# FedeMont/collision_handling_in_instantNGP

Hardware: AMD Instinct MI355X
Metric: Mpixels/sec fwd+bwd at L=16,F=2,T=2^19 (higher is better)
Workload: dtype f32

## Files before the change

collision_handling_in_instantngp_amd/csrc/decoder.hip:

```cpp
#include "gngf_common.h"
#include <type_traits>
#include <utility>

namespace gngf {

using f32x16 = __attribute__((ext_vector_type(16))) float;

constexpr int kH = 64;
constexpr int kDecThreads = 256;

__device__ __forceinline__ int crow(int r, int h) { return (r & 3) + 8 * (r >> 2) + 4 * h; }
__device__ __forceinline__ int kmapC(int s2, int h) { return 32 * (s2 >> 4) + crow(s2 & 15, h); }

__device__ __forceinline__ float vmax0(float z) { float r; asm("v_max_f32 %0, 0, %1" : "=v"(r) : "v"(z)); return r; }
template <bool LEAKY> __device__ __forceinline__ float hidden_act(float z) {
  if (LEAKY) { float r; const float t = 0.01f * z; asm("v_max_f32 %0, %1, %2" : "=v"(r) : "v"(z), "v"(t)); return r; }
  return vmax0(z);
}
template <bool LEAKY> __device__ __forceinline__ float hidden_dsel(float y, float d) { return y > 0.f ? d : (LEAKY ? 0.01f * d : 0.f); }

using f32x2 = __attribute__((ext_vector_type(2))) float;
__device__ __forceinline__ unsigned lds_addr(const float* p) {
  return (unsigned)(size_t)(__attribute__((address_space(3))) const float*)p;
}
// ... 405 lines not shown
  const int64_t ntiles = (P + 127) / 128;
  int64_t zlo = 0, zhi = 0;
  int zper = 0;
  constexpr bool kClears = TRAIN || (KIN == 64 && EXACT && !HYB);
  if constexpr (kClears) {
    if (zero_fill && zero_vecs > 0) {
      const int64_t per = (zero_vecs + gridDim.x - 1) / gridDim.x;
      zlo = (int64_t)blockIdx.x * per + threadIdx.x;
      zhi = (int64_t)(blockIdx.x + 1) * per < zero_vecs ? (int64_t)(blockIdx.x + 1) * per : zero_vecs;
      const int64_t my_tiles = (ntiles - blockIdx.x + gridDim.x - 1) / gridDim.x;
      zper = (int)((per + (int64_t)kDecThreads * my_tiles - 1) / ((int64_t)kDecThreads * my_tiles));
    }
  }
  const unsigned xoff = (unsigned)(((wave * 32 + i) * in_dim + (EXACT ? h * S0 : 0)) * 4);
  const unsigned yoff = (unsigned)(((wave * 32 + i) * out_dim) * 4);
  float xr[S0], yn[4], dyn[4], dz3[4];
  const bool fused_loss = target != nullptr;
  const float* dsrc = fused_loss ? target : dY;
  const float kloss = fused_loss ? gloss[0] * (2.0f / (float)(P * out_dim)) : 0.f;
  auto tile_window = [&](int64_t t, int64_t& tt, int& rows) {
    tt = t < ntiles ? bwd_tile(t, ntiles) : ntiles;
    int64_t rem = P - tt * 128;
    rows = (int)(rem < 0 ? 0 : (rem > 128 ? 128 : rem));
  };
  auto fetch_x = [&](int64_t t) {
    int64_t tt; int rows;
    tile_window(t, tt, rows);
    const __amdgpu_buffer_rsrc_t rx = __builtin_amdgcn_make_buffer_rsrc(const_cast<float*>(X) + tt * 128 * in_dim, 0, rows * in_dim * 4, 0x00020000);
    if (EXACT) {
#pragma unroll
      for (int k = 0; k < S0 / 4; ++k) {
        const u32x4 v = __builtin_amdgcn_raw_buffer_load_b128(rx, xoff + 16 * k, 0, GNGF_BWD_X_AUX);
        xr[4 * k] = __uint_as_float(v.x); xr[4 * k + 1] = __uint_as_float(v.y);
        xr[4 * k + 2] = __uint_as_float(v.z); xr[4 * k + 3] = __uint_as_float(v.w);
      }
    } else {
#pragma unroll
      for (int sx = 0; sx < S0; ++sx) {
        const int k = h * S0 + sx;
        xr[sx] = __uint_as_float(__builtin_amdgcn_raw_buffer_load_b32(rx, k < in_dim ? xoff + 4 * k : 0x40000000u, 0, 0));
      }
    }
  };
  auto fetch_y = [&](int64_t t) {
    int64_t tt; int rows;
    tile_window(t, tt, rows);
    const __amdgpu_buffer_rsrc_t ry = __builtin_amdgcn_make_buffer_rsrc(const_cast<float*>(Yout) + tt * 128 * out_dim, 0, rows * out_dim * 4, 0x00020000);
    const __amdgpu_buffer_rsrc_t rd = __builtin_amdgcn_make_buffer_rsrc(const_cast<float*>(dsrc) + tt * 128 * out_dim, 0, rows * out_dim * 4, 0x00020000);
#pragma unroll
    for (int c = 0; c < 4; ++c) {
      const unsigned off = c < out_dim ? yoff + 4u * c : 0x40000000u;
      if constexpr (!TRAIN) yn[c] = __uint_as_float(__builtin_amdgcn_raw_buffer_load_b32(ry, off, 0, 0));
      dyn[c] = __uint_as_float(__builtin_amdgcn_raw_buffer_load_b32(rd, off, 0, 0));
    }
  };
  auto make_dz3 = [&]() {
#pragma unroll
    for (int c = 0; c < 4; ++c) {
      const float dy = fused_loss ? kloss * (yn[c] - dyn[c]) : dyn[c];
      dz3[c] = dy * (yn[c] * (1.f - yn[c]));
      asm volatile("" : "+v"(dz3[c]));
      db2acc[c] += dz3[c];
    }
  };
  fetch_x(blockIdx.x);
  fetch_y(blockIdx.x);
  if constexpr (!TRAIN) make_dz3();
  float b2v[4] = {0.f, 0.f, 0.f, 0.f};
  if constexpr (TRAIN) {
#pragma unroll
    for (int c = 0; c < 4; ++c) b2v[c] = raw[ro.b2 + c];
  }
  f32x16 b0v[2], b1v[2];
  if (RECOMPUTE) {
#pragma unroll
    for (int t = 0; t < 2; ++t) {
#pragma unroll
      for (int r = 0; r < 16; ++r) { b0v[t][r] = bs[32 * t + crow(r, h)]; b1v[t][r] = bs[kH + 32 * t + crow(r, h)]; }
      asm volatile("" : "+a"(b0v[t]), "+a"(b1v[t]));
    }
  }
  unsigned dxmax = 0u;
#if defined(GNGF_STAMPS)
  unsigned long long ph[10] = {0, 0, 0, 0, 0, 0, 0, 0, 0, 0}, tlast;
  asm volatile("s_memtime %0\n\ts_waitcnt lgkmcnt(0)" : "=s"(tlast) :: "memory");
#endif
  constexpr bool kCarryF0 = KIN <= 32;
  float f0[2][S0];
  f32x16 acc1[2], acc2[2];
  float ft[2][32];
  const unsigned hoff = (unsigned)(wave * 8192 + lane * 16);
  if (!RECOMPUTE && !TRAIN) {
    hidden_load(hidden, blockIdx.x, ntiles, 0, hoff, acc1);
    hidden_load(hidden, blockIdx.x, ntiles, 1, hoff, acc2);
    if constexpr (!HYB) {
#pragma unroll
      for (int s2 = 0; s2 < 32; ++s2) { ft[0][s2] = A1T[(0 * 32 + s2) * 64 + lane]; ft[1][s2] = A1T[(1 * 32 + s2) * 64 + lane]; }
    }
  }
  auto store_hidden_images = [&](auto E) {
    constexpr int e0 = 2 * E.value;
    static_for<2>([&](auto J) {
      constexpr int e = e0 + J.value, t = e >> 4, r = e & 15;
      lds_store<(32 * t + (r & 3) + 8 * (r >> 2)) * kImgStride * 4>(wTile, acc2[t][r]);
      lds_store<kImgB + (32 * t + (r & 3) + 8 * (r >> 2)) * kImgStride * 4>(wTile, acc1[t][r]);
    });
  };
  if constexpr (HYB && !TRAIN) static_for<16>([&](auto E) { store_hidden_images(E); });
  const u32x4* w1t = reinterpret_cast<const u32x4*>(A1T) + lane;
  const u32x4* w0t = reinterpret_cast<const u32x4*>(A0T) + lane;
  Planes w1p[HYB ? 8 : 1], w0p[HYB ? 4 : 1];
  if constexpr (HYB) {
#pragma unroll
    for (int f = 0; f < 8; ++f) {
      w1p[f] = load_planes(w1t + f * 3 * 64);
      asm volatile("" : "+a"(w1p[f].hi), "+a"(w1p[f].mid), "+a"(w1p[f].lo));
    }
  }
  u32x4* w1f = reinterpret_cast<u32x4*>(A1T);
  if constexpr (TRAIN) {
    asm volatile("s_waitcnt lgkmcnt(0)" ::: "memory");
    __syncthreads();
    for (int f = threadIdx.x >> 6; f < 8; f += 4) {
      const int cc = f >> 1, t = f & 1;
      const float* r1 = raw + ro.w1 + (32 * t + i) * 65;
      store_planes(w1f + f * 3 * 64 + lane, split8(r1[kmapS(cc, h, 0)], r1[kmapS(cc, h, 1)], r1[kmapS(cc, h, 2)], r1[kmapS(cc, h, 3)],
                                                  r1[kmapS(cc, h, 4)], r1[kmapS(cc, h, 5)], r1[kmapS(cc, h, 6)], r1[kmapS(cc, h, 7)]));
    }
    __syncthreads();
  }
  if (RECOMPUTE && kCarryF0) {
#pragma unroll
    for (int sx = 0; sx < S0; ++sx) { f0[0][sx] = A0[(0 * S0 + sx) * 64 + lane]; f0[1][sx] = A0[(1 * S0 + sx) * 64 + lane]; }
  }
#define STEP_END() __builtin_amdgcn_sched_barrier(0)
  for (int64_t tile = blockIdx.x; tile < ntiles; tile += gridDim.x) {
    pin_acc();
    STAMP(0);
    float f1[2][32];
    if constexpr (TRAIN) {
      Planes pa0 = load_planes(w0f + lane), pa1 = load_planes(w0f + 3 * 64 + lane);
#pragma unroll
      for (int t = 0; t < 2; ++t)
#pragma unroll
        for (int g = 0; g < 4; ++g) {
          const f32x4 q0 = *reinterpret_cast<const f32x4*>(bs + 32 * t + 8 * g + 4 * h);
          const f32x4 q1 = *reinterpret_cast<const f32x4*>(bs + kH + 32 * t + 8 * g + 4 * h);
#pragma unroll
          for (int e = 0; e < 4; ++e) { acc1[t][4 * g + e] = q0[e]; acc2[t][4 * g + e] = q1[e]; }
        }
      Planes zc = split8(xr[0], xr[1], xr[2], xr[3], xr[4], xr[5], xr[6], xr[7]);
      unsigned nh[4], nm[4], nl[4];
      auto quarter = [&](int q, float a, float b) {
        nh[q] = pack_hi16(b, a);
        const float ra = trunc_residual(a), rb = trunc_residual(b);
        nm[q] = pack_hi16(rb, ra);
        nl[q] = pack_hi16(trunc_residual(rb), trunc_residual(ra));
      };
      auto take_next = [&]() {
        zc.hi = u32x4{nh[0], nh[1], nh[2], nh[3]}; zc.mid = u32x4{nm[0], nm[1], nm[2], nm[3]}; zc.lo = u32x4{nl[0], nl[1], nl[2], nl[3]};
      };
      {
        const Planes na0 = load_planes(w0f + 2 * 3 * 64 + lane), na1 = load_planes(w0f + 3 * 3 * 64 + lane);
        acc1[0] = mfma_b(pa0.hi, zc.lo, acc1[0]);  acc1[1] = mfma_b(pa1.hi, zc.lo, acc1[1]);  quarter(0, xr[8], xr[9]);   STEP_END();
        acc1[0] = mfma_b(pa0.lo, zc.hi, acc1[0]);  acc1[1] = mfma_b(pa1.lo, zc.hi, acc1[1]);  quarter(1, xr[10], xr[11]); STEP_END();
        acc1[0] = mfma_b(pa0.mid, zc.mid, acc1[0]); acc1[1] = mfma_b(pa1.mid, zc.mid, acc1[1]); quarter(2, xr[12], xr[13]); STEP_END();
        acc1[0] = mfma_b(pa0.hi, zc.mid, acc1[0]); acc1[1] = mfma_b(pa1.hi, zc.mid, acc1[1]); quarter(3, xr[14], xr[15]); STEP_END();
        acc1[0] = mfma_b(pa0.mid, zc.hi, acc1[0]); acc1[1] = mfma_b(pa1.mid, zc.hi, acc1[1]);
        acc1[0] = mfma_b(pa0.hi, zc.hi, acc1[0]);  acc1[1] = mfma_b(pa1.hi, zc.hi, acc1[1]);  STEP_END();
        take_next(); pa0 = na0; pa1 = na1;
      }
      {
        const Planes na0 = load_planes(w1f + lane), na1 = load_planes(w1f + 3 * 64 + lane);
        mfma_split2(pa0, pa1, zc, acc1[0], acc1[1]);
        STEP_END();
        pa0 = na0; pa1 = na1;
      }
#pragma unroll
      for (int t = 0; t < 2; ++t)
#pragma unroll
        for (int r = 0; r < 16; ++r) acc1[t][r] = hidden_act<LEAKY>(acc1[t][r]);
      zc = split8(acc1[0][0], acc1[0][1], acc1[0][2], acc1[0][3], acc1[0][4], acc1[0][5], acc1[0][6], acc1[0][7]);
      STEP_END();
      static_for<4>([&](auto CC) {
        constexpr int cc = CC.value, nc = cc + 1;
        Planes na0, na1;
        if constexpr (nc < 4) { na0 = load_planes(w1f + (2 * nc) * 3 * 64 + lane); na1 = load_planes(w1f + (2 * nc + 1) * 3 * 64 + lane); }
        auto step = [&](auto PP, u32x4 a0, u32x4 a1, u32x4 b) {
          constexpr int pp = PP.value;
          acc2[0] = mfma_b(a0, b, acc2[0]);
          acc2[1] = mfma_b(a1, b, acc2[1]);
          if constexpr (nc < 4 && pp < 4) {
            constexpr int t = nc >> 1, r0 = 8 * (nc & 1) + 2 * pp;
            quarter(pp, acc1[t][r0], acc1[t][r0 + 1]);
          }
          if constexpr (pp < 4) {
            static_for<2>([&](auto E) {
              constexpr int e = 8 * cc + 2 * pp + E.value, tt = e >> 4, r = e & 15;
              lds_store<kImgB + (32 * tt + (r & 3) + 8 * (r >> 2)) * kImgStride * 4>(wTile, acc1[tt][r]);
            });
          }
          STEP_END();
        };
        step(std::integral_constant<int, 0>{}, pa0.hi, pa1.hi, zc.lo);
        step(std::integral_constant<int, 1>{}, pa0.lo, pa1.lo, zc.hi);
        step(std::integral_constant<int, 2>{}, pa0.mid, pa1.mid, zc.mid);
        step(std::integral_constant<int, 3>{}, pa0.hi, pa1.hi, zc.mid);
        step(std::integral_constant<int, 4>{}, pa0.mid, pa1.mid, zc.hi);
        step(std::integral_constant<int, 5>{}, pa0.hi, pa1.hi, zc.hi);
        if constexpr (nc < 4) { take_next(); pa0 = na0; pa1 = na1; }
      });
      f32x4 w2v[8];
#pragma unroll
      for (int g = 0; g < 8; ++g) w2v[g] = *reinterpret_cast<const f32x4*>(w2L + (g * 64 + lane) * 4);
#pragma unroll
      for (int t = 0; t < 2; ++t)
#pragma unroll
        for (int r = 0; r < 16; ++r) acc2[t][r] = hidden_act<LEAKY>(acc2[t][r]);
      STEP_END();
      {
        f32x4 o0 = {0.f, 0.f, 0.f, 0.f}, o1 = {0.f, 0.f, 0.f, 0.f};
#pragma unroll
        for (int g = 0; g < 8; ++g) {
          const f32x4 w = w2v[g];
          o0 = __builtin_amdgcn_mfma_f32_4x4x1f32(w.x, acc2[(4 * g) >> 4][(4 * g) & 15], o0, 0, 0, 0);
          o1 = __builtin_amdgcn_mfma_f32_4x4x1f32(w.y, acc2[(4 * g + 1) >> 4][(4 * g + 1) & 15], o1, 0, 0, 0);
          o0 = __builtin_amdgcn_mfma_f32_4x4x1f32(w.z, acc2[(4 * g + 2) >> 4][(4 * g + 2) & 15], o0, 0, 0, 0);
          o1 = __builtin_amdgcn_mfma_f32_4x4x1f32(w.w, acc2[(4 * g + 3) >> 4][(4 * g + 3) & 15], o1, 0, 0, 0);
        }
        int64_t rem = (P - tile * 128) * out_dim * 4;
        rem = rem > 128 * out_dim * 4 ? 128 * out_dim * 4 : rem;
        const __amdgpu_buffer_rsrc_t rs = __builtin_amdgcn_make_buffer_rsrc(const_cast<float*>(Yout) + tile * 128 * out_dim, 0, (int)rem, 0x00020000);
#pragma unroll
        for (int c = 0; c < 4; ++c) {
          const float dc = o0[c] + o1[c];
          const float z = dc + __shfl_xor(dc, 32, 64) + b2v[c];
          const float y = __builtin_amdgcn_rcpf(1.0f + __builtin_amdgcn_exp2f(z * -1.4426950408889634f));
          const unsigned off = (h == 0 && c < out_dim) ? yoff + 4u * c : 0x40000000u;
          __builtin_amdgcn_raw_buffer_store_b32(__float_as_uint(y), rs, off, 0, 0);
          yn[c] = (c < out_dim && tile * 128 + wave * 32 + i < P) ? y : 0.f;
        }
      }
      make_dz3();
      STEP_END();
    }
    if constexpr (RECOMPUTE) {
    if (!kCarryF0) {
#pragma unroll
      for (int sx = 0; sx < S0; ++sx) { f0[0][sx] = A0[(0 * S0 + sx) * 64 + lane]; f0[1][sx] = A0[(1 * S0 + sx) * 64 + lane]; }
      STEP_END();
    }
    static_for<S0>([&](auto SX) {
      constexpr int sx = SX.value;
      if constexpr (sx == 0) { acc1[0] = MFMA(f0[0][0], xr[0], b0v[0]); acc1[1] = MFMA(f0[1][0], xr[0], b0v[1]); }
      else { acc1[0] = MFMA(f0[0][sx], xr[sx], acc1[0]); acc1[1] = MFMA(f0[1][sx], xr[sx], acc1[1]); }
      if (BL::kDedicatedX) lds_store<kImgX + sx * kImgStride * 4>(wX, xr[sx]);
#pragma unroll
      for (int j = 0; j < 64 / S0; ++j) {
        const int e = sx * (64 / S0) + j;
        f1[e >> 5][e & 31] = A1[e * 64 + lane];
      }
      STEP_END();
    });
    if (BL::kDedicatedX) fetch_x(tile + gridDim.x);
#pragma unroll
    for (int t = 0; t < 2; ++t)
#pragma unroll
      for (int r = 0; r < 16; ++r) acc1[t][r] = hidden_act<LEAKY>(acc1[t][r]);
    STEP_END();
    static_for<32>([&](auto S2) {
      constexpr int s2 = S2.value, t = s2 >> 4, r = s2 & 15;
      if constexpr (s2 == 0) { acc2[0] = MFMA(f1[0][0], acc1[0][0], b1v[0]); acc2[1] = MFMA(f1[1][0], acc1[0][0], b1v[1]); }
      else { acc2[0] = MFMA(f1[0][s2], acc1[t][r], acc2[0]); acc2[1] = MFMA(f1[1][s2], acc1[t][r], acc2[1]); }
      lds_store<kImgB + (32 * t + (r & 3) + 8 * (r >> 2)) * kImgStride * 4>(wTile, acc1[t][r]);
      if constexpr (s2 < 4) lds_store<kImgZ + s2 * kImgStride * 4>(wDz3, dz3[s2]);
      ft[0][s2] = A1T[(0 * 32 + s2) * 64 + lane];
      ft[1][s2] = A1T[(1 * 32 + s2) * 64 + lane];
      STEP_END();
    });
    }
    pin_acc();
    STAMP(1);
    f32x16 d2[2];
    {
      float fa[2][2], bsel[2];
#pragma unroll
      for (int sk = 0; sk < 2; ++sk) {
        fa[0][sk] = A2T[(0 * 2 + sk) * 64 + lane]; fa[1][sk] = A2T[(1 * 2 + sk) * 64 + lane];
        float lo = dz3[2 * sk], hi = dz3[2 * sk + 1];
        asm volatile("" : "+v"(lo), "+v"(hi));
        bsel[sk] = h == 0 ? lo : hi;
      }
      STEP_END();
      MFMA_VV_ZERO(d2[0], fa[0][0], bsel[0]); MFMA_VV_ZERO(d2[1], fa[1][0], bsel[0]);
      MFMA_VV(d2[0], fa[0][1], bsel[1]); MFMA_VV(d2[1], fa[1][1], bsel[1]);
      if constexpr (!RECOMPUTE) {
        if (BL::kDedicatedX) static_for<S0>([&](auto SX) { lds_store<kImgX + SX.value * kImgStride * 4>(wX, xr[SX.value]); });
        static_for<4>([&](auto C) { lds_store<kImgZ + C.value * kImgStride * 4>(wDz3, dz3[C.value]); });
      }
    }
    if (!RECOMPUTE && BL::kDedicatedX) fetch_x(tile + gridDim.x);
    fetch_y(tile + gridDim.x);
    MFMA_DRAIN(d2[0], d2[1]);
    STEP_END();
#pragma unroll
    for (int t = 0; t < 2; ++t)
#pragma unroll
      for (int r = 0; r < 16; ++r) {
        if (RECOMPUTE) acc2[t][r] = hidden_act<LEAKY>(acc2[t][r]);
        d2[t][r] = hidden_dsel<LEAKY>(acc2[t][r], d2[t][r]);
      }
    pin_acc();
    STEP_END();
    STAMP(3);
    f32x16 d1[2];
    f32x2 a0p[8], a1p[8], b0p[8], b1p[8];
    float h1v[2][16];
    if constexpr (HYB) {
      f32x2 av[16], bv[16];
      auto lds_step = [&](auto S) {
        constexpr int s2 = S.value;
        if constexpr (s2 < 16) {
          if constexpr (TRAIN) {
            if constexpr (s2 < 8) {
              static_for<4>([&](auto E) {
                constexpr int e = 4 * s2 + E.value, t = e >> 4, r = e & 15;
                lds_store<(32 * t + (r & 3) + 8 * (r >> 2)) * kImgStride * 4>(wTile, acc2[t][r]);
              });
            } else {
              static_for<2>([&](auto E) {
                constexpr int q = 2 * (s2 - 8) + E.value;
                av[q] = lds_load2<kImgZ + 8 * q>(rZ2);
                bv[q] = lds_load2<8 * q>(rH2);
              });
            }
          } else {
            av[s2] = lds_load2<kImgZ + 8 * s2>(rZ2);
            bv[s2] = lds_load2<8 * s2>(rH2);
          }
        } else if constexpr (s2 < 24) {
          static_for<4>([&](auto E) {
            constexpr int e = 4 * (s2 - 16) + E.value, t = e >> 4, r = e & 15;
            lds_store<(32 * t + (r & 3) + 8 * (r >> 2)) * kImgStride * 4>(wTile, d2[t][r]);
          });
        } else {
          constexpr int q = s2 - 24;
          a0p[q] = lds_load2<(2 * q) * 4>(rOp);
          a1p[q] = lds_load2<(32 * kImgStride + 2 * q) * 4>(rOp);
          b0p[q] = lds_load2<kImgB + (2 * q) * 4>(rOp);
          b1p[q] = lds_load2<kImgB + (32 * kImgStride + 2 * q) * 4>(rOp);
        }
      };
      Planes zc = split8(d2[0][0], d2[0][1], d2[0][2], d2[0][3], d2[0][4], d2[0][5], d2[0][6], d2[0][7]);
      d1[0] = 0; d1[1] = 0;
      static_for<4>([&](auto CC) {
        constexpr int cc = CC.value, nc = cc + 1;
        unsigned nh[4], nm[4], nl[4];
        const Planes& fa0 = w1p[2 * cc];
        const Planes& fa1 = w1p[2 * cc + 1];
        auto pair = [&](auto PP, u32x4 a0, u32x4 a1, u32x4 b) {
          constexpr int pp = PP.value;
          d1[0] = mfma_b(a0, b, d1[0]);
          d1[1] = mfma_b(a1, b, d1[1]);
          constexpr int first = 8 * cc + (pp < 1 ? 0 : pp < 4 ? pp + 1 : pp + 2), count = (pp == 0 || pp == 3) ? 2 : 1;
          static_for<count>([&](auto J) { lds_step(std::integral_constant<int, first + J.value>{}); });
          if constexpr (nc < 4) {
            if constexpr (pp < 4) {
              constexpr int t = nc >> 1, r0 = 8 * (nc & 1) + 2 * pp;
              const float a = d2[t][r0], b2 = d2[t][r0 + 1];
              nh[pp] = pack_hi16(b2, a);
              const float ra = trunc_residual(a), rb = trunc_residual(b2);
              nm[pp] = pack_hi16(rb, ra);
              nl[pp] = pack_hi16(trunc_residual(rb), trunc_residual(ra));
            }
          }
          STEP_END();
        };
        pair(std::integral_constant<int, 0>{}, fa0.hi, fa1.hi, zc.lo);
        pair(std::integral_constant<int, 1>{}, fa0.lo, fa1.lo, zc.hi);
        pair(std::integral_constant<int, 2>{}, fa0.mid, fa1.mid, zc.mid);
        pair(std::integral_constant<int, 3>{}, fa0.hi, fa1.hi, zc.mid);
        pair(std::integral_constant<int, 4>{}, fa0.mid, fa1.mid, zc.hi);
        pair(std::integral_constant<int, 5>{}, fa0.hi, fa1.hi, zc.hi);
        if constexpr (nc < 4) {
          zc.hi = u32x4{nh[0], nh[1], nh[2], nh[3]}; zc.mid = u32x4{nm[0], nm[1], nm[2], nm[3]}; zc.lo = u32x4{nl[0], nl[1], nl[2], nl[3]};
        }
        if constexpr (cc == 1) {
          lds_wait();
#pragma unroll
          for (int q = 0; q < 16; ++q) {
            dW2acc = __builtin_amdgcn_mfma_f32_4x4x1f32(av[q].x, bv[q].x, dW2acc, 0, 0, 0);
            dW2acc = __builtin_amdgcn_mfma_f32_4x4x1f32(av[q].y, bv[q].y, dW2acc, 0, 0, 0);
          }
          STEP_END();
        }
      });
    } else {
    {
      f32x2 av[16], bv[16];
      static_for<16>([&](auto S2) {
        constexpr int s2 = S2.value;
        if constexpr (s2 == 0) { MFMA_VV_ZERO(d1[0], ft[0][0], d2[0][0]); MFMA_VV_ZERO(d1[1], ft[1][0], d2[0][0]); }
        else { MFMA_VV(d1[0], ft[0][s2], d2[0][s2]); MFMA_VV(d1[1], ft[1][s2], d2[0][s2]); }
        if constexpr (s2 < 8) {
          static_for<4>([&](auto E) {
            constexpr int e = 4 * s2 + E.value, t = e >> 4, r = e & 15;
            lds_store<(32 * t + (r & 3) + 8 * (r >> 2)) * kImgStride * 4>(wTile, acc2[t][r]);
            if constexpr (!RECOMPUTE)
              lds_store<kImgB + (32 * t + (r & 3) + 8 * (r >> 2)) * kImgStride * 4>(wTile, acc1[t][r]);
          });
        } else {
          static_for<2>([&](auto E) {
            constexpr int q = 2 * (s2 - 8) + E.value;
            av[q] = lds_load2<kImgZ + 8 * q>(rZ2);
            bv[q] = lds_load2<8 * q>(rH2);
          });
        }
        STEP_END();
      });
      lds_wait();
#pragma unroll
      for (int q = 0; q < 16; ++q) {
        dW2acc = __builtin_amdgcn_mfma_f32_4x4x1f32(av[q].x, bv[q].x, dW2acc, 0, 0, 0);
        dW2acc = __builtin_amdgcn_mfma_f32_4x4x1f32(av[q].y, bv[q].y, dW2acc, 0, 0, 0);
      }
      STEP_END();
    }
    static_for<16>([&](auto S2) {
      constexpr int s2 = 16 + S2.value, k = S2.value;
      MFMA_VV(d1[0], ft[0][s2], d2[1][k]);
      MFMA_VV(d1[1], ft[1][s2], d2[1][k]);
      if constexpr (k < 8) {
        static_for<4>([&](auto E) {
          constexpr int e = 4 * k + E.value, t = e >> 4, r = e & 15;
          lds_store<(32 * t + (r & 3) + 8 * (r >> 2)) * kImgStride * 4>(wTile, d2[t][r]);
        });
      } else {
        constexpr int q = k - 8;
        a0p[q] = lds_load2<(2 * q) * 4>(rOp);
        a1p[q] = lds_load2<(32 * kImgStride + 2 * q) * 4>(rOp);
        b0p[q] = lds_load2<kImgB + (2 * q) * 4>(rOp);
        b1p[q] = lds_load2<kImgB + (32 * kImgStride + 2 * q) * 4>(rOp);
        if constexpr (RECOMPUTE)
          static_for<4>([&](auto E) {
            constexpr int e = 4 * q + E.value, t = e >> 4, r = e & 15;
            h1v[t][r] = lds_load1<kImgB + (32 * t + (r & 3) + 8 * (r >> 2)) * kImgStride * 4>(wTile);
          });
      }
      STEP_END();
    });
    MFMA_DRAIN(d1[0], d1[1]);
    }
    lds_wait();
#pragma unroll
    for (int t = 0; t < 2; ++t)
#pragma unroll
      for (int r = 0; r < 16; ++r) d1[t][r] = hidden_dsel<LEAKY>(RECOMPUTE ? h1v[t][r] : acc1[t][r], d1[t][r]);
    {
      f32x2 s0 = a0p[0], s1 = a1p[0];
#pragma unroll
      for (int q = 1; q < 8; ++q) { s0 += a0p[q]; s1 += a1p[q]; }
      db1acc[0] += s0.x + s0.y; db1acc[1] += s1.x + s1.y;
    }
    if (!RECOMPUTE && !TRAIN) {
      STEP_END();
      hidden_load(hidden, tile + gridDim.x, ntiles, 1, hoff, acc2);
    }
    pin_acc();
    STEP_END();
    STAMP(5);
    f32x2 c0p[8], c1p[8], xp[TX][8];
    float fx[TX][32];
    static_for<8>([&](auto Q) {
      constexpr int q = Q.value;
      if constexpr (HYB && !TRAIN && q == 0) hidden_load(hidden, tile + gridDim.x, ntiles, 0, hoff, acc1);
      dW1acc[0][0] = MFMA(a0p[q].x, b0p[q].x, dW1acc[0][0]);
      dW1acc[0][1] = MFMA(a0p[q].x, b1p[q].x, dW1acc[0][1]);
      dW1acc[1][0] = MFMA(a1p[q].x, b0p[q].x, dW1acc[1][0]);
      dW1acc[1][1] = MFMA(a1p[q].x, b1p[q].x, dW1acc[1][1]);
      dW1acc[0][0] = MFMA(a0p[q].y, b0p[q].y, dW1acc[0][0]);
      dW1acc[0][1] = MFMA(a0p[q].y, b1p[q].y, dW1acc[0][1]);
      dW1acc[1][0] = MFMA(a1p[q].y, b0p[q].y, dW1acc[1][0]);
      dW1acc[1][1] = MFMA(a1p[q].y, b1p[q].y, dW1acc[1][1]);
      if constexpr (q < 4) {
        static_for<8>([&](auto E) {
          constexpr int e = 8 * q + E.value, t = e >> 4, r = e & 15;
          lds_store<(32 * t + (r & 3) + 8 * (r >> 2)) * kImgStride * 4>(wTile, d1[t][r]);
        });
        if constexpr (!BL::kDedicatedX)
          static_for<S0 / 4>([&](auto E) { constexpr int sx = q * (S0 / 4) + E.value; lds_store<kImgX + sx * kImgStride * 4>(wX, xr[sx]); });
      } else {
        static_for<2>([&](auto E) {
          constexpr int qq = 2 * (q - 4) + E.value;
          c0p[qq] = lds_load2<(2 * qq) * 4>(rOp);
          c1p[qq] = lds_load2<(32 * kImgStride + 2 * qq) * 4>(rOp);
          xp[0][qq] = lds_load2<kImgX + (2 * qq) * 4>(rOp);
          if constexpr (TX > 1) xp[TX - 1][qq] = lds_load2<kImgX + (32 * kImgStride + 2 * qq) * 4>(rOp);
        });
        if constexpr (!HYB) {
#pragma unroll
          for (int j = 0; j < 8; ++j) fx[0][8 * (q - 4) + j] = A0T[(8 * (q - 4) + j) * 64 + lane];
        }
        if (kCarryF0 && TX > 1) {
#pragma unroll
          for (int j = 0; j < 8; ++j) fx[TX - 1][8 * (q - 4) + j] = A0T[((TX - 1) * 32 + 8 * (q - 4) + j) * 64 + lane];
        }
      }
      STEP_END();
    });
    if (!BL::kDedicatedX) fetch_x(tile + gridDim.x);
    lds_wait();
    pin_acc();
    STAMP(4);
    static_for<8>([&](auto Q) {
      constexpr int q = Q.value;
#pragma unroll
      for (int tx = 0; tx < TX; ++tx) {
        dW0acc[0][tx] = MFMA(c0p[q].x, xp[tx][q].x, dW0acc[0][tx]);
        dW0acc[1][tx] = MFMA(c1p[q].x, xp[tx][q].x, dW0acc[1][tx]);
        dW0acc[0][tx] = MFMA(c0p[q].y, xp[tx][q].y, dW0acc[0][tx]);
        dW0acc[1][tx] = MFMA(c1p[q].y, xp[tx][q].y, dW0acc[1][tx]);
      }
      if constexpr (!RECOMPUTE && !HYB && q == 0) hidden_load(hidden, tile + gridDim.x, ntiles, 0, hoff, acc1);
      if constexpr (HYB) {
        if constexpr (!TRAIN) {
          store_hidden_images(std::integral_constant<int, 2 * q>{});
          store_hidden_images(std::integral_constant<int, 2 * q + 1>{});
        }
        if constexpr (q >= 2 && q < 6) w0p[q - 2] = load_planes(w0t + (q - 2) * 3 * 64);
      }
      if (RECOMPUTE && kCarryF0) {
#pragma unroll
        for (int j = 0; j < 2 * S0 / 8; ++j) {
          const int e = q * (2 * S0 / 8) + j;
          f0[e / S0][e % S0] = A0[e * 64 + lane];
        }
      } else if (!kCarryF0 && TX > 1) {
#pragma unroll
        for (int j = 0; j < 4; ++j) fx[TX - 1][4 * q + j] = A0T[((TX - 1) * 32 + 4 * q + j) * 64 + lane];
      }
      STEP_END();
    });
    pin_acc();
    STAMP(6);
    f32x16 dxv[TX];
    if constexpr (HYB) {
      f32x16 acc;
      acc = 0;
      Planes zc = split8(d1[0][0], d1[0][1], d1[0][2], d1[0][3], d1[0][4], d1[0][5], d1[0][6], d1[0][7]);
      static_for<4>([&](auto CC) {
        constexpr int cc = CC.value, nc = cc + 1;
        Planes nz;
        const Planes& fa = w0p[cc];
        if constexpr (nc < 4) {
          constexpr int t = nc >> 1, r0 = 8 * (nc & 1);
          nz = split8(d1[t][r0], d1[t][r0 + 1], d1[t][r0 + 2], d1[t][r0 + 3], d1[t][r0 + 4], d1[t][r0 + 5], d1[t][r0 + 6], d1[t][r0 + 7]);
        }
        acc = mfma_b(fa.hi, zc.lo, acc);
        acc = mfma_b(fa.lo, zc.hi, acc);
        acc = mfma_b(fa.mid, zc.mid, acc);
        acc = mfma_b(fa.hi, zc.mid, acc);
        acc = mfma_b(fa.mid, zc.hi, acc);
        acc = mfma_b(fa.hi, zc.hi, acc);
        STEP_END();
        if constexpr (nc < 4) zc = nz;
      });
      dxv[0] = acc;
    } else {
#pragma unroll
    for (int tx = 0; tx < TX; ++tx) {
      MFMA_VV_ZERO(dxv[tx], fx[tx][0], d1[0][0]);
#pragma unroll
      for (int s2 = 1; s2 < 32; ++s2) {
        MFMA_VV(dxv[tx], fx[tx][s2], d1[s2 >> 4][s2 & 15]);
        if (!RECOMPUTE && tx == TX - 1) {
          ft[0][s2] = A1T[(0 * 32 + s2) * 64 + lane];
          ft[1][s2] = A1T[(1 * 32 + s2) * 64 + lane];
          if (s2 == 1) { ft[0][0] = A1T[lane]; ft[1][0] = A1T[32 * 64 + lane]; }
        }
      }
    }
    if constexpr (TX > 1) MFMA_DRAIN(dxv[0], dxv[TX - 1]);
    else MFMA_DRAIN1(dxv[0]);
    }
    STEP_END();
#pragma unroll
    for (int tx = 0; tx < TX; ++tx)
#pragma unroll
      for (int r = 0; r < 16; ++r) {
        const unsigned a = __float_as_uint(dxv[tx][r]) & 0x7fffffffu;
        dxmax = a > dxmax ? a : dxmax;
      }
    {
      f32x2 s0 = c0p[0], s1 = c1p[0];
#pragma unroll
      for (int q = 1; q < 8; ++q) { s0 += c0p[q]; s1 += c1p[q]; }
      db0acc[0] += s0.x + s0.y; db0acc[1] += s1.x + s1.y;
    }
    if constexpr (!TRAIN) make_dz3();
    STEP_END();
    {
      const int64_t pt = bwd_tile(tile, ntiles);
      int64_t rem = P - pt * 128;
      rem = rem > 128 ? 128 : rem;
      const __amdgpu_buffer_rsrc_t rs = __builtin_amdgcn_make_buffer_rsrc(dX + pt * 128 * in_dim, 0, (int)rem * in_dim * 4, 0x00020000);
      const unsigned base = (unsigned)((wave * 32 + i) * in_dim) * 4u;
#pragma unroll
      for (int tx = 0; tx < TX; ++tx)
#pragma unroll
        for (int g = 0; g < 4; ++g) {
          const int col = 32 * tx + 8 * g + 4 * h;
          if (EXACT) {
            if (32 * tx + 8 * g + 8 <= KIN) {
              u32x4 v = {__float_as_uint(dxv[tx][4 * g]), __float_as_uint(dxv[tx][4 * g + 1]), __float_as_uint(dxv[tx][4 * g + 2]),
                         __float_as_uint(dxv[tx][4 * g + 3])};
              __builtin_amdgcn_raw_buffer_store_b128(v, rs, base + 4u * col, 0, 0);
            }
          } else {
#pragma unroll
            for (int q = 0; q < 4; ++q)
              __builtin_amdgcn_raw_buffer_store_b32(__float_as_uint(dxv[tx][4 * g + q]), rs, col + q < in_dim ? base + 4u * (col + q) : 0x40000000u, 0, 0);
          }
        }
    }
    if constexpr (kClears) {
      for (int z = 0; z < zper; ++z, zlo += kDecThreads)
        if (zlo < zhi) zero_fill[zlo] = float4{0.f, 0.f, 0.f, 0.f};
    }
    pin_acc();
    STEP_END();
    STAMP(7);
  }

#if defined(GNGF_STAMPS)
  if (blockIdx.x == 7 && threadIdx.x == 0)
    for (int k = 0; k < 10; ++k) g_stamps[k] = ph[k];
  if (threadIdx.x == 0) g_blocktime[1][blockIdx.x & 255][1] = __builtin_readcyclecounter();
#endif
#pragma unroll
  for (int o = 32; o > 0; o >>= 1) { const unsigned ov = (unsigned)__shfl_xor((int)dxmax, o, 64); dxmax = ov > dxmax ? ov : dxmax; }
  __syncthreads();
  float* region = smem + wave * nslab;
  float* sW0 = region;
  float* sW1 = sW0 + kH * in_dim;
  float* sW2 = sW1 + kH * kH;
  float* sb0 = sW2 + out_dim * kH;
  float* sb1 = sb0 + kH;
  float* sb2 = sb1 + kH;
#pragma unroll
  for (int ti = 0; ti < 2; ++ti)
#pragma unroll
    for (int r = 0; r < 16; ++r) {
      const int row = 32 * ti + crow(r, h);
#pragma unroll
      for (int tj = 0; tj < 2; ++tj) sW1[row * kH + 32 * tj + i] = dW1acc[ti][tj][r];
#pragma unroll
      for (int tx = 0; tx < TX; ++tx)
        if (32 * tx + i < in_dim) sW0[row * in_dim + 32 * tx + i] = dW0acc[ti][tx][r];
    }
#pragma unroll
  for (int ti = 0; ti < 2; ++ti) {
    const float v0 = db0acc[ti] + __shfl_xor(db0acc[ti], 32, 64), v1 = db1acc[ti] + __shfl_xor(db1acc[ti], 32, 64);
    if (h == 0) { sb0[32 * ti + i] = v0; sb1[32 * ti + i] = v1; }
  }
#pragma unroll
  for (int c = 0; c < 4; ++c)
    if (c < out_dim) sW2[c * kH + lane] = dW2acc[c];
#pragma unroll
  for (int c = 0; c < 4; ++c) {
    float v = h == 0 ? db2acc[c] : 0.f;
#pragma unroll
    for (int o = 32; o > 0; o >>= 1) v += __shfl_xor(v, o, 64);
    if (lane == 0 && c < out_dim) sb2[c] = v;
  }
  if (lane == 0) region[nslab - 1] = __uint_as_float(dxmax);
  __syncthreads();
  float* out = slabs + (int64_t)blockIdx.x * nslab;
  for (int e = threadIdx.x; e < nslab - 1; e += kDecThreads)
    out[e] = (smem[e] + smem[nslab + e]) + (smem[2 * nslab + e] + smem[3 * nslab + e]);
  if (threadIdx.x == 0) {
    unsigned mx = 0u;
#pragma unroll
    for (int w = 0; w < 4; ++w) { const unsigned v = __float_as_uint(smem[w * nslab + nslab - 1]); mx = v > mx ? v : mx; }
    out[nslab - 1] = __uint_as_float(mx);
    atomicMax(&g_bwd_span[1], (unsigned long long)wall_clock64());
  }
}

__global__ void __launch_bounds__(1024)
decoder_reduce_kernel(const float* __restrict__ slabs, int nslabs, int nslab, int in_dim, int out_dim,
                      float* __restrict__ dW0, float* __restrict__ db0, float* __restrict__ dW1, float* __restrict__ db1,
                      float* __restrict__ dW2, float* __restrict__ db2, float* __restrict__ absmax,
                      const float* __restrict__ promised, const float* __restrict__ arrived) {
  decoder_reduce_block(blockIdx.x, slabs, nslabs, nslab, in_dim, out_dim, dW0, db0, dW1, db1, dW2, db2, absmax, promised, arrived);
}

template <int KIN>
static size_t bwd_smem_bytes(int in_dim, int out_dim) {
  using FF = FwdFrags<KIN>;
  constexpr int TX = (KIN + 31) / 32;
  const int img = 4 * BwdLds<KIN>::kWaveFloats, slab = slab_size(in_dim, out_dim);
  const size_t main_loop = (size_t)(FF::kA0 + FF::kA1 + 2 * 2 * 64 + 2 * 32 * 64 + TX * 32 * 64 + 2 * kH + img);
  const size_t epilogue = (size_t)4 * slab;
  return sizeof(float) * (main_loop > epilogue ? main_loop : epilogue);
}
static size_t bwd_smem_bytes_hybrid(int out_dim) {
  using FF = FwdFrags<32>;
  const int img = 4 * BwdLds<32>::kWaveFloats, slab = slab_size(32, out_dim);
  const size_t main_loop = (size_t)(FF::kA0 + FF::kA1 + 2 * 2 * 64 + 12 * 3 * 64 * 4 + 2 * kH + img);
  const size_t epilogue = (size_t)4 * slab;
  return sizeof(float) * (main_loop > epilogue ? main_loop : epilogue);
}
static int g_decoder_bwd_hybrid = 1;

}

using namespace gngf;

extern "C" int gngf_set_decoder_bwd_hybrid(int on) {
// ... 169 lines not shown
```

collision_handling_in_instantngp_amd/csrc/decoder_split.inc:

```

struct Planes { u32x4 hi, mid, lo; };

__device__ __forceinline__ unsigned pack_hi16(float b, float a) {
  return __builtin_amdgcn_perm(__float_as_uint(b), __float_as_uint(a), 0x07060302u);
}
__device__ __forceinline__ float trunc_residual(float v) { return v - __uint_as_float(__float_as_uint(v) & 0xffff0000u); }

__device__ __forceinline__ Planes split8(float x0, float x1, float x2, float x3, float x4, float x5, float x6, float x7) {
  const float x[8] = {x0, x1, x2, x3, x4, x5, x6, x7};
  unsigned hi[4], mid[4], lo[4];
#pragma unroll
  for (int q = 0; q < 4; ++q) {
    const float a = x[2 * q], b = x[2 * q + 1];
    hi[q] = pack_hi16(b, a);
    const float ra = trunc_residual(a), rb = trunc_residual(b);
    mid[q] = pack_hi16(rb, ra);
    lo[q] = pack_hi16(trunc_residual(rb), trunc_residual(ra));
  }
  Planes p;
  p.hi = u32x4{hi[0], hi[1], hi[2], hi[3]}; p.mid = u32x4{mid[0], mid[1], mid[2], mid[3]}; p.lo = u32x4{lo[0], lo[1], lo[2], lo[3]};
  return p;
}

using bf16x8_t = __attribute__((ext_vector_type(8))) __bf16;
__device__ __forceinline__ f32x16 mfma_b(u32x4 a, u32x4 b, f32x16 c) {
  return __builtin_amdgcn_mfma_f32_32x32x16_bf16(__builtin_bit_cast(bf16x8_t, a), __builtin_bit_cast(bf16x8_t, b), c, 0, 0, 0);
}
__device__ __forceinline__ void mfma_split2(const Planes& a0, const Planes& a1, const Planes& b, f32x16& c0, f32x16& c1) {
  c0 = mfma_b(a0.hi, b.lo, c0);  c1 = mfma_b(a1.hi, b.lo, c1);
  c0 = mfma_b(a0.lo, b.hi, c0);  c1 = mfma_b(a1.lo, b.hi, c1);
  c0 = mfma_b(a0.mid, b.mid, c0); c1 = mfma_b(a1.mid, b.mid, c1);
  c0 = mfma_b(a0.hi, b.mid, c0); c1 = mfma_b(a1.hi, b.mid, c1);
  c0 = mfma_b(a0.mid, b.hi, c0); c1 = mfma_b(a1.mid, b.hi, c1);
  c0 = mfma_b(a0.hi, b.hi, c0);  c1 = mfma_b(a1.hi, b.hi, c1);
}

__device__ __forceinline__ int kmapS(int cc, int h, int j) { return 32 * (cc >> 1) + crow(8 * (cc & 1) + j, h); }

__device__ __forceinline__ void store_planes(u32x4* dst, const Planes& p) { dst[0] = p.hi; dst[64] = p.mid; dst[128] = p.lo; }
__device__ __forceinline__ Planes load_planes(const u32x4* src) { Planes p; p.hi = src[0]; p.mid = src[64]; p.lo = src[128]; return p; }
```

Before: 2605.

## Interleave split-bf16 packing and activations into MFMA issue slots in train path

Reorders the TRAIN-path MLP forward and backward so that the split-bf16 plane packing, ReLU activations and derivative selects are spread across twelve fine-grained slots between individual MFMAs, using sched barriers and register pins. Layer-0 work is reordered to finish one accumulator before the other, so its activation and split can overlap the remaining MFMAs. The bias-gradient reduction is folded into the final dx MFMA chain. The goal is to hide VALU work under MFMA latency, at the cost of much more rigid hand scheduling and possible extra register pressure.

New measurement: 2653, median of 6. 1.02x the previous value.

```diff
diff --git a/collision_handling_in_instantngp_amd/csrc/decoder.hip b/collision_handling_in_instantngp_amd/csrc/decoder.hip
--- a/collision_handling_in_instantngp_amd/csrc/decoder.hip
+++ b/collision_handling_in_instantngp_amd/csrc/decoder.hip
@@ -511,7 +511,8 @@
   }
   unsigned dxmax = 0u;
 #if defined(GNGF_STAMPS)
-  unsigned long long ph[10] = {0, 0, 0, 0, 0, 0, 0, 0, 0, 0}, tlast;
+  unsigned ph[16] = {0, 0, 0, 0, 0, 0, 0, 0, 0, 0, 0, 0, 0, 0, 0, 0};
+  unsigned long long tlast;
   asm volatile("s_memtime %0\n\ts_waitcnt lgkmcnt(0)" : "=s"(tlast) :: "memory");
 #endif
   constexpr bool kCarryF0 = KIN <= 32;
@@ -563,6 +564,9 @@
     for (int sx = 0; sx < S0; ++sx) { f0[0][sx] = A0[(0 * S0 + sx) * 64 + lane]; f0[1][sx] = A0[(1 * S0 + sx) * 64 + lane]; }
   }
 #define STEP_END() __builtin_amdgcn_sched_barrier(0)
+#define SLOT_END() __builtin_amdgcn_sched_barrier(0)
+#define SLOT_END1(x) do { asm volatile("" : "+a"(x)); __builtin_amdgcn_sched_barrier(0); } while (0)
+#define SLOT_END2(x, y) do { asm volatile("" : "+a"(x), "+a"(y)); __builtin_amdgcn_sched_barrier(0); } while (0)
   for (int64_t tile = blockIdx.x; tile < ntiles; tile += gridDim.x) {
     pin_acc();
     STAMP(0);
@@ -579,74 +583,95 @@
           for (int e = 0; e < 4; ++e) { acc1[t][4 * g + e] = q0[e]; acc2[t][4 * g + e] = q1[e]; }
         }
       Planes zc = split8(xr[0], xr[1], xr[2], xr[3], xr[4], xr[5], xr[6], xr[7]);
+      STAMP(8);
       unsigned nh[4], nm[4], nl[4];
-      auto quarter = [&](int q, float a, float b) {
-        nh[q] = pack_hi16(b, a);
-        const float ra = trunc_residual(a), rb = trunc_residual(b);
-        nm[q] = pack_hi16(rb, ra);
-        nl[q] = pack_hi16(trunc_residual(rb), trunc_residual(ra));
-      };
-      auto take_next = [&]() {
-        zc.hi = u32x4{nh[0], nh[1], nh[2], nh[3]}; zc.mid = u32x4{nm[0], nm[1], nm[2], nm[3]}; zc.lo = u32x4{nl[0], nl[1], nl[2], nl[3]};
+      float sra, srb;
+      auto next_planes = [&]() {
+        Planes p;
+        p.hi = u32x4{nh[0], nh[1], nh[2], nh[3]}; p.mid = u32x4{nm[0], nm[1], nm[2], nm[3]}; p.lo = u32x4{nl[0], nl[1], nl[2], nl[3]};
+        return p;
       };
       {
-        const Planes na0 = load_planes(w0f + 2 * 3 * 64 + lane), na1 = load_planes(w0f + 3 * 3 * 64 + lane);
-        acc1[0] = mfma_b(pa0.hi, zc.lo, acc1[0]);  acc1[1] = mfma_b(pa1.hi, zc.lo, acc1[1]);  quarter(0, xr[8], xr[9]);   STEP_END();
-        acc1[0] = mfma_b(pa0.lo, zc.hi, acc1[0]);  acc1[1] = mfma_b(pa1.lo, zc.hi, acc1[1]);  quarter(1, xr[10], xr[11]); STEP_END();
-        acc1[0] = mfma_b(pa0.mid, zc.mid, acc1[0]); acc1[1] = mfma_b(pa1.mid, zc.mid, acc1[1]); quarter(2, xr[12], xr[13]); STEP_END();
-        acc1[0] = mfma_b(pa0.hi, zc.mid, acc1[0]); acc1[1] = mfma_b(pa1.hi, zc.mid, acc1[1]); quarter(3, xr[14], xr[15]); STEP_END();
-        acc1[0] = mfma_b(pa0.mid, zc.hi, acc1[0]); acc1[1] = mfma_b(pa1.mid, zc.hi, acc1[1]);
-        acc1[0] = mfma_b(pa0.hi, zc.hi, acc1[0]);  acc1[1] = mfma_b(pa1.hi, zc.hi, acc1[1]);  STEP_END();
-        take_next(); pa0 = na0; pa1 = na1;
-      }
-      {
+        const Planes pb0 = load_planes(w0f + 2 * 3 * 64 + lane), pb1 = load_planes(w0f + 3 * 3 * 64 + lane);
+        static_for<6>([&](auto S) {
+          constexpr int s = S.value;
+          static_for<2>([&](auto J) {
+            constexpr int k = 2 * s + J.value;
+            split_twelfth<k>(xr[8 + 2 * (k / 3)], xr[9 + 2 * (k / 3)], nh, nm, nl, sra, srb);
+          });
+          mfma_cross<s>(pa0, zc, acc1[0]);
+          SLOT_END1(acc1[0]);
+        });
+        const Planes zn = next_planes();
+        static_for<6>([&](auto S) { mfma_cross<S.value>(pb0, zn, acc1[0]); SLOT_END1(acc1[0]); });
         const Planes na0 = load_planes(w1f + lane), na1 = load_planes(w1f + 3 * 64 + lane);
-        mfma_split2(pa0, pa1, zc, acc1[0], acc1[1]);
-        STEP_END();
-        pa0 = na0; pa1 = na1;
-      }
-#pragma unroll
-      for (int t = 0; t < 2; ++t)
-#pragma unroll
-        for (int r = 0; r < 16; ++r) acc1[t][r] = hidden_act<LEAKY>(acc1[t][r]);
-      zc = split8(acc1[0][0], acc1[0][1], acc1[0][2], acc1[0][3], acc1[0][4], acc1[0][5], acc1[0][6], acc1[0][7]);
-      STEP_END();
+        static_for<12>([&](auto S) {
+          constexpr int s = S.value;
+          if constexpr (s < 6) mfma_cross<s>(pa1, zc, acc1[1]);
+          else mfma_cross<s - 6>(pb1, zn, acc1[1]);
+          SLOT_END1(acc1[1]);
+          constexpr int r_lo[12] = {0, 3, 6, 9, 10, 11, 11, 12, 12, 13, 13, 14}, r_hi[12] = {3, 6, 9, 10, 11, 11, 12, 12, 13, 13, 14, 16};
+          constexpr int k_lo[12] = {0, 0, 0, 1, 2, 3, 5, 6, 8, 9, 11, 12}, k_hi[12] = {0, 0, 1, 2, 3, 5, 6, 8, 9, 11, 12, 12};
+          static_for<r_hi[s] - r_lo[s]>([&](auto R) {
+            constexpr int r = r_lo[s] + R.value;
+            acc1[0][r] = hidden_act<LEAKY>(acc1[0][r]);
+            asm volatile("" : "+v"(acc1[0][r]));
+          });
+          static_for<k_hi[s] - k_lo[s]>([&](auto K) {
+            constexpr int k = k_lo[s] + K.value;
+            split_twelfth<k>(acc1[0][2 * (k / 3)], acc1[0][2 * (k / 3) + 1], nh, nm, nl, sra, srb);
+          });
+          SLOT_END();
+        });
+        zc = next_planes(); pa0 = na0; pa1 = na1;
+      }
+      STAMP(2);
+      STAMP(9);
       static_for<4>([&](auto CC) {
         constexpr int cc = CC.value, nc = cc + 1;
         Planes na0, na1;
         if constexpr (nc < 4) { na0 = load_planes(w1f + (2 * nc) * 3 * 64 + lane); na1 = load_planes(w1f + (2 * nc + 1) * 3 * 64 + lane); }
-        auto step = [&](auto PP, u32x4 a0, u32x4 a1, u32x4 b) {
-          constexpr int pp = PP.value;
-          acc2[0] = mfma_b(a0, b, acc2[0]);
-          acc2[1] = mfma_b(a1, b, acc2[1]);
-          if constexpr (nc < 4 && pp < 4) {
-            constexpr int t = nc >> 1, r0 = 8 * (nc & 1) + 2 * pp;
-            quarter(pp, acc1[t][r0], acc1[t][r0 + 1]);
+        static_for<12>([&](auto S) {
+          constexpr int s = S.value;
+          constexpr int t = nc < 4 ? (s & 1) : s / 6, pp = nc < 4 ? (s >> 1) : s % 6;
+          if constexpr (nc < 4) {
+            constexpr int tn = nc >> 1, r0 = 8 * (nc & 1) + 2 * (s / 3);
+            split_twelfth<s>(acc1[tn][r0], acc1[tn][r0 + 1], nh, nm, nl, sra, srb);
           }
-          if constexpr (pp < 4) {
+          if constexpr (t == 0) mfma_cross<pp>(pa0, zc, acc2[0]);
+          else mfma_cross<pp>(pa1, zc, acc2[1]);
+          if constexpr (s < 8) {
+            constexpr int e = 8 * cc + s, tt = e >> 4, r = e & 15;
+            lds_store<kImgB + (32 * tt + (r & 3) + 8 * (r >> 2)) * kImgStride * 4>(wTile, acc1[tt][r]);
+          }
+          if constexpr (cc < 2 && s % 3 == 0)
             static_for<2>([&](auto E) {
-              constexpr int e = 8 * cc + 2 * pp + E.value, tt = e >> 4, r = e & 15;
-              lds_store<kImgB + (32 * tt + (r & 3) + 8 * (r >> 2)) * kImgStride * 4>(wTile, acc1[tt][r]);
+              constexpr int r = 8 * cc + 2 * (s / 3) + E.value;
+              acc1[1][r] = hidden_act<LEAKY>(acc1[1][r]);
+              asm volatile("" : "+v"(acc1[1][r]));
             });
+          if constexpr (nc == 4 && s >= 6) SLOT_END1(acc2[1]);
+          else SLOT_END2(acc2[0], acc2[1]);
+          if constexpr (nc == 4 && s >= 6) {
+            constexpr int r_lo = s < 10 ? 3 * (s - 6) : 12 + 2 * (s - 10), n = s < 10 ? 3 : 2;
+            static_for<n>([&](auto R) {
+              constexpr int r = r_lo + R.value;
+              acc2[0][r] = hidden_act<LEAKY>(acc2[0][r]);
+              asm volatile("" : "+v"(acc2[0][r]));
+            });
+            SLOT_END();
           }
-          STEP_END();
-        };
-        step(std::integral_constant<int, 0>{}, pa0.hi, pa1.hi, zc.lo);
-        step(std::integral_constant<int, 1>{}, pa0.lo, pa1.lo, zc.hi);
-        step(std::integral_constant<int, 2>{}, pa0.mid, pa1.mid, zc.mid);
-        step(std::integral_constant<int, 3>{}, pa0.hi, pa1.hi, zc.mid);
-        step(std::integral_constant<int, 4>{}, pa0.mid, pa1.mid, zc.hi);
-        step(std::integral_constant<int, 5>{}, pa0.hi, pa1.hi, zc.hi);
-        if constexpr (nc < 4) { take_next(); pa0 = na0; pa1 = na1; }
+        });
+        if constexpr (nc < 4) { zc = next_planes(); pa0 = na0; pa1 = na1; }
       });
+      STAMP(10);
       f32x4 w2v[8];
 #pragma unroll
       for (int g = 0; g < 8; ++g) w2v[g] = *reinterpret_cast<const f32x4*>(w2L + (g * 64 + lane) * 4);
 #pragma unroll
-      for (int t = 0; t < 2; ++t)
-#pragma unroll
-        for (int r = 0; r < 16; ++r) acc2[t][r] = hidden_act<LEAKY>(acc2[t][r]);
+      for (int r = 0; r < 16; ++r) acc2[1][r] = hidden_act<LEAKY>(acc2[1][r]);
       STEP_END();
+      STAMP(11);
       {
         f32x4 o0 = {0.f, 0.f, 0.f, 0.f}, o1 = {0.f, 0.f, 0.f, 0.f};
 #pragma unroll
@@ -732,6 +757,11 @@
     fetch_y(tile + gridDim.x);
     MFMA_DRAIN(d2[0], d2[1]);
     STEP_END();
+    STAMP(12);
+    if constexpr (TRAIN) {
+#pragma unroll
+      for (int r = 0; r < 8; ++r) d2[0][r] = hidden_dsel<LEAKY>(acc2[0][r], d2[0][r]);
+    } else {
 #pragma unroll
     for (int t = 0; t < 2; ++t)
 #pragma unroll
@@ -739,6 +769,7 @@
         if (RECOMPUTE) acc2[t][r] = hidden_act<LEAKY>(acc2[t][r]);
         d2[t][r] = hidden_dsel<LEAKY>(acc2[t][r], d2[t][r]);
       }
+    }
     pin_acc();
     STEP_END();
     STAMP(3);
@@ -782,6 +813,54 @@
       };
       Planes zc = split8(d2[0][0], d2[0][1], d2[0][2], d2[0][3], d2[0][4], d2[0][5], d2[0][6], d2[0][7]);
       d1[0] = 0; d1[1] = 0;
+      STAMP(13);
+      if constexpr (TRAIN) {
+      static_for<4>([&](auto CC) {
+        constexpr int cc = CC.value, nc = cc + 1;
+        unsigned nh[4], nm[4], nl[4];
+        float sra, srb;
+        static_for<12>([&](auto S) {
+          constexpr int s = S.value;
+          constexpr int t = nc < 4 ? (s & 1) : s / 6, pp = nc < 4 ? (s >> 1) : s % 6;
+          if constexpr (nc < 4) {
+            constexpr int tn = nc >> 1, r0 = 8 * (nc & 1) + 2 * (s / 3);
+            if constexpr (s % 3 == 0) {
+              d2[tn][r0] = hidden_dsel<LEAKY>(acc2[tn][r0], d2[tn][r0]);
+              d2[tn][r0 + 1] = hidden_dsel<LEAKY>(acc2[tn][r0 + 1], d2[tn][r0 + 1]);
+            }
+            split_twelfth<s>(d2[tn][r0], d2[tn][r0 + 1], nh, nm, nl, sra, srb);
+          }
+          mfma_cross<pp>(w1p[2 * cc + t], zc, d1[t]);
+          if constexpr ((s & 1) == 0) {
+            constexpr int lp = s >> 1;
+            constexpr int first = 8 * cc + (lp < 1 ? 0 : lp < 4 ? lp + 1 : lp + 2), count = (lp == 0 || lp == 3) ? 2 : 1;
+            static_for<count>([&](auto J) { lds_step(std::integral_constant<int, first + J.value>{}); });
+          }
+          if constexpr (nc == 4 && s >= 6) SLOT_END1(d1[1]);
+          else SLOT_END2(d1[0], d1[1]);
+          if constexpr (nc == 4 && s >= 6) {
+            constexpr int r_lo = s < 10 ? 3 * (s - 6) : 12 + 2 * (s - 10), n = s < 10 ? 3 : 2;
+            static_for<n>([&](auto R) {
+              constexpr int r = r_lo + R.value;
+              d1[0][r] = hidden_dsel<LEAKY>(acc1[0][r], d1[0][r]);
+            });
+            SLOT_END();
+          }
+        });
+        if constexpr (nc < 4) {
+          zc.hi = u32x4{nh[0], nh[1], nh[2], nh[3]}; zc.mid = u32x4{nm[0], nm[1], nm[2], nm[3]}; zc.lo = u32x4{nl[0], nl[1], nl[2], nl[3]};
+        }
+        if constexpr (cc == 1) {
+          lds_wait();
+#pragma unroll
+          for (int q = 0; q < 16; ++q) {
+            dW2acc = __builtin_amdgcn_mfma_f32_4x4x1f32(av[q].x, bv[q].x, dW2acc, 0, 0, 0);
+            dW2acc = __builtin_amdgcn_mfma_f32_4x4x1f32(av[q].y, bv[q].y, dW2acc, 0, 0, 0);
+          }
+          STEP_END();
+        }
+      });
+      } else
       static_for<4>([&](auto CC) {
         constexpr int cc = CC.value, nc = cc + 1;
         unsigned nh[4], nm[4], nl[4];
@@ -824,6 +903,7 @@
           STEP_END();
         }
       });
+      STAMP(14);
     } else {
     {
       f32x2 av[16], bv[16];
@@ -884,7 +964,9 @@
 #pragma unroll
     for (int t = 0; t < 2; ++t)
 #pragma unroll
-      for (int r = 0; r < 16; ++r) d1[t][r] = hidden_dsel<LEAKY>(RECOMPUTE ? h1v[t][r] : acc1[t][r], d1[t][r]);
+      for (int r = 0; r < 16; ++r)
+        if (!(TRAIN && t == 0))
+          d1[t][r] = hidden_dsel<LEAKY>(RECOMPUTE ? h1v[t][r] : acc1[t][r], d1[t][r]);
     {
       f32x2 s0 = a0p[0], s1 = a1p[0];
 #pragma unroll
@@ -985,16 +1067,29 @@
           constexpr int t = nc >> 1, r0 = 8 * (nc & 1);
           nz = split8(d1[t][r0], d1[t][r0 + 1], d1[t][r0 + 2], d1[t][r0 + 3], d1[t][r0 + 4], d1[t][r0 + 5], d1[t][r0 + 6], d1[t][r0 + 7]);
         }
+        if constexpr (TRAIN && nc == 4) {
+          f32x2 s0 = c0p[0], s1 = c1p[0];
+          static_for<6>([&](auto PP) {
+            constexpr int p = PP.value;
+            mfma_cross<p>(fa, zc, acc);
+            s0 += c0p[p + 1]; s1 += c1p[p + 1];
+            if constexpr (p == 5) { s0 += c0p[7]; s1 += c1p[7]; db0acc[0] += s0.x + s0.y; db0acc[1] += s1.x + s1.y; }
+            else asm volatile("" : "+v"(s0), "+v"(s1));
+            SLOT_END1(acc);
+          });
+        } else {
         acc = mfma_b(fa.hi, zc.lo, acc);
         acc = mfma_b(fa.lo, zc.hi, acc);
         acc = mfma_b(fa.mid, zc.mid, acc);
         acc = mfma_b(fa.hi, zc.mid, acc);
         acc = mfma_b(fa.mid, zc.hi, acc);
         acc = mfma_b(fa.hi, zc.hi, acc);
+        }
         STEP_END();
         if constexpr (nc < 4) zc = nz;
       });
       dxv[0] = acc;
+      STAMP(15);
     } else {
 #pragma unroll
     for (int tx = 0; tx < TX; ++tx) {
@@ -1020,13 +1115,13 @@
         const unsigned a = __float_as_uint(dxv[tx][r]) & 0x7fffffffu;
         dxmax = a > dxmax ? a : dxmax;
       }
-    {
+    if constexpr (!TRAIN) {
       f32x2 s0 = c0p[0], s1 = c1p[0];
 #pragma unroll
       for (int q = 1; q < 8; ++q) { s0 += c0p[q]; s1 += c1p[q]; }
       db0acc[0] += s0.x + s0.y; db0acc[1] += s1.x + s1.y;
-    }
-    if constexpr (!TRAIN) make_dz3();
+      make_dz3();
+    }
     STEP_END();
     {
       const int64_t pt = bwd_tile(tile, ntiles);
@@ -1063,7 +1158,7 @@
 
 #if defined(GNGF_STAMPS)
   if (blockIdx.x == 7 && threadIdx.x == 0)
-    for (int k = 0; k < 10; ++k) g_stamps[k] = ph[k];
+    for (int k = 0; k < 16; ++k) g_stamps[k] = ph[k];
   if (threadIdx.x == 0) g_blocktime[1][blockIdx.x & 255][1] = __builtin_readcyclecounter();
 #endif
 #pragma unroll
diff --git a/collision_handling_in_instantngp_amd/csrc/decoder_split.inc b/collision_handling_in_instantngp_amd/csrc/decoder_split.inc
--- a/collision_handling_in_instantngp_amd/csrc/decoder_split.inc
+++ b/collision_handling_in_instantngp_amd/csrc/decoder_split.inc
@@ -35,6 +35,24 @@
   c0 = mfma_b(a0.hi, b.hi, c0);  c1 = mfma_b(a1.hi, b.hi, c1);
 }
 
+template <int P> __device__ __forceinline__ void mfma_cross(const Planes& a, const Planes& b, f32x16& c) {
+  static_assert(P >= 0 && P < 6, "six cross terms");
+  if constexpr (P == 0) c = mfma_b(a.hi, b.lo, c);
+  else if constexpr (P == 1) c = mfma_b(a.lo, b.hi, c);
+  else if constexpr (P == 2) c = mfma_b(a.mid, b.mid, c);
+  else if constexpr (P == 3) c = mfma_b(a.hi, b.mid, c);
+  else if constexpr (P == 4) c = mfma_b(a.mid, b.hi, c);
+  else c = mfma_b(a.hi, b.hi, c);
+}
+template <int K> __device__ __forceinline__ void split_twelfth(float a, float b, unsigned (&hi)[4], unsigned (&mid)[4], unsigned (&lo)[4],
+                                                              float& ra, float& rb) {
+  constexpr int q = K / 3, p = K % 3;
+  static_assert(K >= 0 && K < 12, "twelve sub-steps");
+  if constexpr (p == 0) { hi[q] = pack_hi16(b, a); asm volatile("" : "+v"(hi[q])); }
+  else if constexpr (p == 1) { ra = trunc_residual(a); rb = trunc_residual(b); mid[q] = pack_hi16(rb, ra); asm volatile("" : "+v"(mid[q])); }
+  else { lo[q] = pack_hi16(trunc_residual(rb), trunc_residual(ra)); asm volatile("" : "+v"(lo[q])); }
+}
+
 __device__ __forceinline__ int kmapS(int cc, int h, int j) { return 32 * (cc >> 1) + crow(8 * (cc & 1) + j, h); }
 
 __device__ __forceinline__ void store_planes(u32x4* dst, const Planes& p) { dst[0] = p.hi; dst[64] = p.mid; dst[128] = p.lo; }
```
